# Ai00-X/ai00_server

Measured on NVIDIA H100. Metric: decode tokens/s RWKV-6-World-7B fp16 batch=16, higher is better.
Workload: dtype f16

## Files before the change

### ai00_server_b200/csrc/engine.cu

```cuda
#include "../../include/b200rwkv.h"

#include <unistd.h>

#include <algorithm>
#include <condition_variable>
#include <functional>
#include <thread>
#include <cmath>
#include <cstdio>
#include <cstdlib>
#include <cstring>
#include <map>
#include <memory>
#include <mutex>
#include <set>
#include <stdexcept>
#include <string>
#include <utility>
#include <vector>

#include "gemm.cuh"
#include "qgemm.cuh"
#include "pre6.cuh"
#include "sample.cuh"
// ... 572 lines not shown
    uint32_t ad_targets = 0;
    std::vector<AdLayer> ad_layers;
    GemmLaunch ad_head;
    AdapterParams s_head;
    int* d_slot_adapter = nullptr;
    std::vector<int> slot_adapter;
    struct AdMatrix {
        std::string name;
        int N, K;
        uint8_t* W;
        int tiles, KB, kbw;
        AdapterParams* sp;
        int proj;
        __half* A[AD_MAX];
    };
    std::vector<AdMatrix> ad_mats;
    std::vector<char> place_full;
    std::map<std::string, StTensor> model_shapes;
    uint8_t* ad_stage = nullptr;
    size_t ad_stage_cols = 0;
    void set_place_rank(const AdMatrix& m, int id, int r);
    void load_place(int id, const StFile& f, float alpha);
    void unload_place(int id);
    void drop_adapter_graphs();
    bool step_bound(const std::vector<int>& slots) const {
        for (int s : slots)
            if (n_adapters && s >= 0 && s < S && slot_adapter[s]) return true;
        return false;
    }
    GemmLaunch ad_launch(const GemmLaunch& base, AdapterParams& sp);
    void enqueue_shrink(const AdapterParams& p, const StepShape& sh, cudaStream_t s, Profiler* prof);
    void check_loras(const StFile& model) const;
    void blend_loras(const StTensor& t);

    Buf<__half> d_tmp;
    const StTensor* d_tmp_holds = nullptr;

    ~b200rwkv_engine();
    void* dalloc(size_t bytes, bool zero = true);
    void build(const StFile& st);
    const __half* upload_tmp(const StTensor& t);
    float* vec_f32(const StFile& st, const std::string& name, size_t off, size_t count, float scale = 1.f, float bias = 0.f);
    A16Buf a16_alloc(int K, int nmat = 1);
    GemmLaunch make_launch(std::vector<SegDesc>& segs, int force_grid = 0, int qtype = QT_NONE);
    int quant_layers = 0, quant_type = QT_NONE;
    int pick_split(int K, int tiles) const;
    void finalize_tp();
    template <typename P, typename... X>
    void launch_k(void (*kern)(P, X...), dim3 grid, dim3 block, size_t smem, const P& params, int cls, cudaStream_t s, Profiler* prof,
                  X... extra);
    bool split_on = false;
    bool split_act = false;
    bool ln_cluster_ok = false;
    unsigned* pre_gbar = nullptr;
    int launch_cluster = 0;
    unsigned long long* d_step_trace = nullptr;
    std::vector<int> step_trace_types;
    static constexpr int STEP_TRACE_MAX = 1024;
    static constexpr int STEP_TRACE_ROW = 512;
    bool trace_capture = false;
    std::vector<long long> step_trace_bytes;
    unsigned long long* tr_next(int label) {
        if (!d_step_trace || !trace_capture || launches_last_step >= STEP_TRACE_MAX) return nullptr;
        if ((int)step_trace_types.size() <= launches_last_step) step_trace_types.resize(launches_last_step + 1);
        step_trace_types[launches_last_step] = label;
        return d_step_trace + (size_t)STEP_TRACE_ROW * launches_last_step;
    }
    StepShape step_shape(int T, int R) const;
    void launch_gemm(const GemmLaunch& g, const StepShape& sh, cudaStream_t s, Profiler* prof, bool head = false);
    void launch_wkv(const WkvParams& p, const StepShape& sh, cudaStream_t s, Profiler* prof);
    LnPick launch_embed(const EmbedParams& p, const StepShape& sh, cudaStream_t s, Profiler* prof);
    LnPick launch_ln(const LnMixParams& p, const StepShape& sh, cudaStream_t s, Profiler* prof);
    LnPick launch_pre6(const Pre6Params& q, const StepShape& sh, cudaStream_t s, Profiler* prof);
    LnPick launch_ln_out(const LnOutParams& p, const StepShape& sh, cudaStream_t s, Profiler* prof);
    void enqueue_step(cudaStream_t s, const StepShape& sh, Profiler* prof);
    void run_step(const StepShape& sh);
    int fill_meta(int* m, const std::vector<int>& slots, const std::vector<int>& counts, const std::vector<const uint32_t*>& toks,
                  const std::vector<int>& outmode , int* R_out);
    struct ScoreOut { float* score; uint32_t* argmax; };
    void infer(int nslot, const int32_t* slot, const int32_t* ntok, const uint32_t* tokens, const int32_t* option,
               float* logits_out, size_t cap, int32_t* rows_out, const ScoreOut* score = nullptr, const SnapPlan* snap = nullptr);
    void state_xform(int slot, bool import, float* snap = nullptr);
};

b200rwkv_engine::~b200rwkv_engine() {
    cudaSetDevice(dev);
    cudaDeviceSynchronize();
    for (int q = 0; q < 8; ++q)
        if (peer_ipc[q] && peer_base[q]) cudaIpcCloseMemHandle(peer_base[q]);
}

void* b200rwkv_engine::dalloc(size_t bytes, bool zero) {
    bytes = std::max<size_t>(bytes, 16);
    allocs.emplace_back(bytes);
    if (zero) CK(cudaMemset(allocs.back(), 0, bytes));
    return allocs.back();
}

const __half* b200rwkv_engine::upload_tmp(const StTensor& t) {
    if (d_tmp_holds != &t) {
        REQUIRE(t.nbytes <= d_tmp.bytes, B200RWKV_ERR_INVALID, "internal: temp buffer too small");
        CK(cudaMemcpy(d_tmp, t.data, t.nbytes, cudaMemcpyHostToDevice));
        d_tmp_holds = &t;
        blend_loras(t);
    }
    return d_tmp;
}
// ... 401 lines not shown
    REQUIRE(H % world == 0 && F % (8 * world) == 0 && V % world == 0, B200RWKV_ERR_UNSUPPORTED,
            "heads / hidden / vocab do not shard evenly over the tensor-parallel world");
    Cl = C / world; Hl = H / world; Fl = F / world; Vl = V / world;
    const int ver = info.version;
    const int c0 = rank * Cl, f0 = rank * Fl, v0 = rank * Vl;

    stream = new_stream();
    sm_stream = new_stream();
    if (quant_layers > 0 && quant_type != QT_NONE) {
        REQUIRE(quant_type == QT_INT8 || quant_type == QT_NF4, B200RWKV_ERR_UNSUPPORTED, "quant_type must be Int8 or NF4 (SF4 is not implemented)");
        REQUIRE(world == 1, B200RWKV_ERR_UNSUPPORTED, "quantised layers are single-GPU in this version");
        REQUIRE(precision == 0, B200RWKV_ERR_UNSUPPORTED, "quantised layers run with precision 0 (f16 operands)");
    }
    gemm_smem_limits(quant_layers > 0 ? quant_type : (int)QT_NONE);
    wkv_smem_limits();
    if (precision == 1) split_act = true;

    meta_ints = MetaView::ints(maxT, S);
    d_meta = (int*)dalloc(meta_ints * 4);
    h_meta = HostBuf<int>(meta_ints * 4 * META_RING);
    memset(h_meta, 0, meta_ints * 4 * META_RING);
    for (auto& ev : meta_ev) ev = new_event(cudaEventDisableTiming);
    MetaView mv{d_meta, maxT, S};

    size_t tmp_bytes = 0;
    for (auto& kv : st.tensors) tmp_bytes = std::max(tmp_bytes, kv.second.nbytes);
    d_tmp = Buf<__half>(tmp_bytes);

    att_shift = (float*)dalloc((size_t)L * S * C * 4);
    ffn_shift = (float*)dalloc((size_t)L * S * C * 4);
    wkv_state = (float*)dalloc((size_t)L * S * Hl * N * N * 4);
    d_api = (float*)dalloc((size_t)L * (N + 2) * C * 4);
    state_from_st(st, L, H, N, C, init_state);

    const size_t TC = (size_t)maxT * C, TCl = (size_t)maxT * Cl;
    x_a = (float*)dalloc(TC * 4); x_b = (float*)dalloc(TC * 4);
    xx1 = (float*)dalloc(TC * 4); sx1 = (float*)dalloc(TC * 4); xx2 = (float*)dalloc(TC * 4);
    f_r = (float*)dalloc(TCl * 4); f_k = (float*)dalloc(TCl * 4); f_v = (float*)dalloc(TCl * 4); f_g = (float*)dalloc(TCl * 4);
    f_w = (float*)dalloc(TCl * 4); f_a = (float*)dalloc(TCl * 4); f_nu = (float*)dalloc(TCl * 4); f_vfirst = (float*)dalloc(TCl * 4);
    {
        auto al = [](size_t x) { return (x + 255) & ~(size_t)255; };
        off_part_att = 0;
        off_part_ffn = al(off_part_att + TC * 4 * 8);
        off_rr = al(off_part_ffn + TC * 4 * 8);
        off_logits = al(off_rr + TCl * 4);
        off_flags = al(off_logits + (size_t)maxT * Vl * 4);
        comm_bytes = al(off_flags + 256);
        comm_base = (uint8_t*)dalloc(comm_bytes, true);
        part_att = (float*)(comm_base + off_part_att);
        part_ffn = (float*)(comm_base + off_part_ffn);
        f_rr = (float*)(comm_base + off_rr);
        d_logits = (float*)(comm_base + off_logits);
        d_epoch = (unsigned*)dalloc(16, true);
        pre_gbar = (unsigned*)dalloc(256, true);
        ln_cluster_ok = ln_cluster_fits(C);
        split_on = split_act && ln_cluster_ok;
        REQUIRE(precision != 1 || split_on, B200RWKV_ERR_UNSUPPORTED, "precision 1 needs num_emb to be a multiple of 32 and <= 8192");
    }
    const int S_att = pick_split(Cl, cdiv(C, GEMM_BN)), S_ffn = pick_split(Fl, cdiv(C, GEMM_BN));
    split_att = S_att; split_ffn = S_ffn;
    d_hidden = (float*)dalloc(TC * 4);
    d_hid_tab = (float**)dalloc((size_t)L * sizeof(float*));
    step_done = new_event(cudaEventDisableTiming);
    keep_valid.assign(S, 0);
    if (rank == 0) {
        d_keep = (float*)dalloc((size_t)S * V * 4);
        const int nseg = cdiv(V, TOPK_SEG);
        if (nseg <= TOPK_MAX_SEGS) {
            tk_cand_x = (float*)dalloc((size_t)S * nseg * TOPK_MAX * 4);
            tk_cand_id = (unsigned*)dalloc((size_t)S * nseg * TOPK_MAX * 4);
            tk_stats = (float2*)dalloc((size_t)S * nseg * 8);
            tk_out_id = (unsigned*)dalloc((size_t)S * TOPK_MAX * 4);
            tk_out_p = (float*)dalloc((size_t)S * TOPK_MAX * 4);
        }
    }
    auto op_cols = [&](int K) { return n_adapters ? (cdiv(K, GEMM_BK) + n_adapters) * GEMM_BK : K; };
    for (int i = 0; i < 6; ++i) a_x[i] = a16_alloc(op_cols(C));
    a_out = a16_alloc(op_cols(Cl));
    a_kk = a16_alloc(op_cols(Fl));
    a_head = a16_alloc(op_cols(C));
    slot_adapter.assign(S, 0);
    if (n_adapters) d_slot_adapter = (int*)dalloc((size_t)S * 4, true);

    {
        const StTensor& e = st.get("emb.weight");
        emb = (__half*)dalloc(e.nbytes, false);
        CK(cudaMemcpy(emb, e.data, e.nbytes, cudaMemcpyHostToDevice));
        embed.emb = emb; embed.C = C; embed.V = V; embed.meta = mv;
        embed.ln_w = vec_f32(st, "blocks.0.ln0.weight", 0, C);
        embed.ln_b = vec_f32(st, "blocks.0.ln0.bias", 0, C);
        embed.x_out = x_a;
    }

    auto base_ln = [&](LnMixParams& p) {
        memset(&p, 0, sizeof(p));
        p.C = C; p.meta = mv;
    };
    auto f32_seg = [&](const StTensor& t, int n0, int Nn, int k0, int K, const A16Buf& ab, float* out, int ldo, int act,
                       const float* bias, int a_koff = 0, int a_mat = 0) {
        SegDesc d;
        d.t = &t; d.n0 = n0; d.N = Nn; d.k0 = k0; d.K = K;
        REQUIRE(a_koff % GEMM_BK == 0, B200RWKV_ERR_INVALID, "internal: split-K slices start on k-block boundaries");
        d.proto.A = ab.p + (size_t)a_mat * ab.halves_per_matrix + (size_t)(a_koff / GEMM_BK) * A16_KB_HALVES;
        d.proto.out_mode = OUT_F32; d.proto.act = act; d.proto.bias = bias; d.proto.out = out; d.proto.ldo = ldo;
        return d;
    };
    auto a16_seg = [&](const StTensor& t, int n0, int Nn, int k0, int K, const A16Buf& ab, const A16Buf& dst, int act,
// ... 47 lines not shown
            if (l == 0) {
                a_lora[0] = a16_alloc(Dm, 5);
                a_lora[1] = a16_alloc(Dd);
            }
            n1.n_mix = 1;
            n1.mu[0] = vec_f32(st, a + "time_mix_x", 0, C);
            n1.mix_out[0] = a_x[5].p;
            n1.sx_out = sx1;
            {
                std::vector<SegDesc> sv;
                SegDesc d = a16_seg(st.get(a + "time_mix_w1"), 0, 5 * Dm, 0, C, a_x[5], a_lora[0], ACT_TANH, nullptr);
                d.proto.grp = Dm;
                d.proto.grp_stride = (int)a_lora[0].halves_per_matrix;
                sv.push_back(d);
                ly.lora.push_back(make_launch(sv));
            }
            static const char* names[5] = {"time_mix_w", "time_mix_k", "time_mix_v", "time_mix_r", "time_mix_g"};
            const float* mu5[5];
            for (int i = 0; i < 5; ++i) mu5[i] = vec_f32(st, a + names[i], 0, C);
            {
                std::vector<SegDesc> sv;
                for (int i = 0; i < 5; ++i) {
                    SegDesc d;
                    d.t = &st.get(a + "time_mix_w2"); d.slice = i; d.n0 = 0; d.N = C; d.k0 = 0; d.K = Dm;
                    d.proto.A = a_lora[0].p + (size_t)i * a_lora[0].halves_per_matrix;
                    d.proto.out_mode = OUT_LERP_A16; d.proto.act = ACT_NONE;
                    d.proto.out = a_x[i].p;
                    d.proto.aux0 = xx1; d.proto.aux1 = sx1; d.proto.aux2 = mu5[i]; d.proto.ld_aux = C;
                    sv.push_back(d);
                }
                ly.lora.push_back(make_launch(sv));
            }
            {
                const StTensor& w1 = st.get(a + "time_mix_w1");
                const StTensor& w2 = st.get(a + "time_mix_w2");
                const StTensor& d2 = st.get(a + "time_decay_w2");
                REQUIRE(w1.shape.size() == 2 && w1.shape[0] == 5 * Dm && w1.shape[1] == C, B200RWKV_ERR_INVALID, "time_mix_w1 must be [5*Dm, C]");
                REQUIRE(w2.shape.size() == 3 && w2.shape[0] == 5 && w2.shape[1] == C && w2.shape[2] == Dm, B200RWKV_ERR_INVALID,
                        "time_mix_w2 must be [5, C, Dm]");
                REQUIRE(d2.shape.size() == 2 && d2.shape[0] == C && d2.shape[1] == Dd, B200RWKV_ERR_INVALID, "time_decay_w2 must be [C, Dd]");
            }
            if (pre6_fits(Dm, C)) {
                auto upload_raw = [&](const StTensor& t) {
                    __half* d = (__half*)dalloc(t.nbytes, false);
                    CK(cudaMemcpy(d, t.data, t.nbytes, cudaMemcpyHostToDevice));
                    return d;
                };
                Pre6Params& q = ly.pre6;
                q.W1 = upload_raw(st.get(a + "time_mix_w1"));
                q.W2 = upload_raw(st.get(a + "time_mix_w2"));
                for (int i = 0; i < 5; ++i) { q.mu[i] = mu5[i]; q.out[i] = a_x[i].p; }
                q.lora = a_lora[0].p; q.lora_stride = (int)a_lora[0].halves_per_matrix;
                q.Dm = Dm;
                q.gbar = pre_gbar;
                ly.has_pre6 = true;
            }
            {
                std::vector<SegDesc> sv;
                sv.push_back(f32_seg(Wr, c0, Cl, 0, C, a_x[3], f_r, Cl, ACT_NONE, nullptr));
                sv.push_back(f32_seg(Wk, c0, Cl, 0, C, a_x[1], f_k, Cl, ACT_NONE, nullptr));
                sv.push_back(f32_seg(Wv, c0, Cl, 0, C, a_x[2], f_v, Cl, ACT_NONE, nullptr));
                sv.push_back(f32_seg(st.get(a + "gate.weight"), c0, Cl, 0, C, a_x[4], f_g, Cl, ACT_SILU, nullptr));
                if (lq != QT_NONE) {
                    std::vector<SegDesc> sd;
                    sd.push_back(a16_seg(st.get(a + "time_decay_w1"), 0, Dd, 0, C, a_x[0], a_lora[1], ACT_TANH, nullptr));
                    ly.pre.push_back(make_launch(sd));
                    ly.pre.push_back(make_launch(sv, 0, lq));
                } else {
                    sv.push_back(a16_seg(st.get(a + "time_decay_w1"), 0, Dd, 0, C, a_x[0], a_lora[1], ACT_TANH, nullptr));
                    ly.pre.push_back(make_launch(sv));
                }
            }
            const float* time_decay = vec_f32(st, a + "time_decay", c0, Cl);
            if (Dd <= 128 && Dd % 8 == 0) {
                const StTensor& t = st.get(a + "time_decay_w2");
                const std::vector<__half> tmp = wd2_k_major(reinterpret_cast<const __half*>(t.data), c0, Hl, Dd);
                __half* dw = (__half*)dalloc(tmp.size() * 2, false);
                CK(cudaMemcpy(dw, tmp.data(), tmp.size() * 2, cudaMemcpyHostToDevice));
                wk.wd2t = dw;
                wk.decay_bias = time_decay;
                wk.d1 = a_lora[1].p;
                wk.Dd = Dd;
            } else {
                std::vector<SegDesc> sv;
                sv.push_back(f32_seg(st.get(a + "time_decay_w2"), c0, Cl, 0, Dd, a_lora[1], f_w, Cl, ACT_EXPNEGEXP, time_decay));
                ly.pre.push_back(make_launch(sv));
            }
            wk.w = f_w;
            wk.u = vec_f32(st, a + "time_first", c0, Cl);
        } else if (ver == 5) {
            static const char* names[4] = {"time_mix_k", "time_mix_v", "time_mix_r", "time_mix_g"};
            n1.n_mix = 4;
            for (int i = 0; i < 4; ++i) {
                n1.mu[i] = vec_f32(st, a + names[i], 0, C, -1.f, 1.f);
                n1.mix_out[i] = a_x[1 + i].p;
            }
            std::vector<SegDesc> sv;
            sv.push_back(f32_seg(Wr, c0, Cl, 0, C, a_x[3], f_r, Cl, ACT_NONE, nullptr));
            sv.push_back(f32_seg(Wk, c0, Cl, 0, C, a_x[1], f_k, Cl, ACT_NONE, nullptr));
            sv.push_back(f32_seg(Wv, c0, Cl, 0, C, a_x[2], f_v, Cl, ACT_NONE, nullptr));
            sv.push_back(f32_seg(st.get(a + "gate.weight"), c0, Cl, 0, C, a_x[4], f_g, Cl, ACT_SILU, nullptr));
            ly.pre.push_back(make_launch(sv, 0, lq));
            {
                const StTensor& td = st.get(a + "time_decay");
                REQUIRE(td.numel() == C, B200RWKV_ERR_UNSUPPORTED, "v5 time_decay must be [H, N]");
                float* d = (float*)dalloc((size_t)Cl * 4, false);
                Buf<__half> tmp((size_t)Cl * 2);
// ... 1917 lines not shown
                "gate blocks (C / n_gate columns) must be whole multiples of 4 columns");
        REQUIRE(!x.commit_src == !x.commit_dst, B200RWKV_ERR_INVALID, "the commit needs both commit_src and commit_dst");
    }
    if (stage == 1 || stage == 2) {
        REQUIRE(x.n_mix >= 1 && x.n_mix <= 6, B200RWKV_ERR_INVALID, "n_mix must be 1..6");
        REQUIRE(x.shift_state && x.mu && x.mix_out && x.xx_out, B200RWKV_ERR_INVALID, "null shift_state, mu, mix_out or xx_out");
        REQUIRE(x.x_out || x.n_parts == 0, B200RWKV_ERR_INVALID, "in place (x_out NULL) takes no parts");
    }
    if (stage == 2) {
        REQUIRE(T <= 16 && pre6_fits(x.Dm, C), B200RWKV_ERR_UNSUPPORTED,
                "the front half runs decode-shaped steps (T <= 16) with Dm 32 or 64, C % 128 == 0 and C <= 4096");
        REQUIRE(x.n_mix == 1 && x.sx_out && x.W1 && x.W2 && x.mu5 && x.lora_out && x.out5, B200RWKV_ERR_INVALID,
                "the front half needs n_mix 1, sx_out, W1, W2, mu5, lora_out and out5");
    }
    std::vector<int> outmode(x.nslot, 0);
    if (stage == 3) {
        REQUIRE(x.option && x.head_out, B200RWKV_ERR_INVALID, "ln_out needs option and head_out");
        for (int i = 0; i < x.nslot; ++i) {
            REQUIRE(x.option[i] >= B200RWKV_OPTION_LAST && x.option[i] <= B200RWKV_OPTION_NONE, B200RWKV_ERR_INVALID, "bad option");
            outmode[i] = x.option[i] == B200RWKV_OPTION_FULL ? 2 : (x.option[i] == B200RWKV_OPTION_LAST ? 1 : 0);
        }
    }
    snap_args_ok(x.nsnap, x.snap_tok, x.snap_rec, x.snap_ld, x.snap_off, C, T);
    if (x.nsnap > 0) {
        REQUIRE(stage != 0, B200RWKV_ERR_INVALID, "the embed stage takes no snapshots");
        REQUIRE(NL == 1, B200RWKV_ERR_INVALID, "snapshots take one launch");
        REQUIRE(stage != 3 || (x.commit_src && x.snap_head_out), B200RWKV_ERR_INVALID, "ln_out snapshots need the commit and snap_head_out");
    }

    st.start(device, NL, x.tokens, outmode);
    float* d_rec = x.nsnap > 0 ? st.snap_start(x.nsnap, x.snap_tok, x.snap_rec, x.snap_ld) : nullptr;
    b200rwkv_engine* e = st.e.get();
    e->ln_cluster_ok = ln_cluster_fits(C);
    const StepShape& sh = st.sh;
    const int th = sh.th;
    const int hrows = std::max(sh.th_rows, 16);
    const int xrows = sh.split ? 32 : 16 * sh.MTX;

    auto rows_down = [&](float* h, const float* d) { CK(cudaMemcpy(h, d, (size_t)T * C * 4, cudaMemcpyDeviceToHost)); };
    auto a16_up = [&](const uint16_t* h, int nmat, int K, int tr) {
        const std::vector<uint16_t> b = a16_pack(h, nmat * K, K, tr, (size_t)tr * K, K);
        return (__half*)st.up(b.data(), b.size() * 2);
    };
    auto a16_down = [&](uint16_t* h, const __half* d, int nmat, int K, int tr) {
        std::vector<uint16_t> b(a16_halves(K) * nmat);
        CK(cudaMemcpy(b.data(), d, b.size() * 2, cudaMemcpyDeviceToHost));
        a16_unpack(b, nmat * K, K, tr, tr, (size_t)tr * K, K, h);
    };

    const size_t TC = (size_t)T * C;
    const float* ln_w = (const float*)st.up(x.ln_w, (size_t)C * 4);
    const float* ln_b = (const float*)st.up(x.ln_b, (size_t)C * 4);
    float* cdst = x.commit_dst ? (float*)st.up(x.commit_dst, (size_t)S * C * 4) : nullptr;
    unsigned* gbar = (unsigned*)e->dalloc(256, true);
    float** hid_tab = nullptr;
    std::vector<float*> hid_rows(NL, nullptr);
    const int gcl = x.n_gate > 0 ? C / x.n_gate : 0;
    auto residual = [&](auto& p, int l) {
        p.x_in = st.rows_up(x.x_in + l * TC, C);
        p.C = C;
        p.meta = st.meta(l);
        p.n_parts = x.n_parts;
        for (int q = 0; q < x.n_parts; ++q) p.parts[q] = st.rows_up(x.parts + ((size_t)l * x.n_parts + q) * TC, C);
        p.n_gate = x.n_gate;
        p.gate_cl = gcl;
        for (int q = 0; q < x.n_gate; ++q) p.gates[q] = st.rows_up(x.gates + ((size_t)l * x.n_gate + q) * T * gcl, gcl);
        p.ln_w = ln_w; p.ln_b = ln_b;
        p.commit_dst = cdst;
        p.commit_src = x.commit_src ? st.rows_up(x.commit_src + l * TC, C) : nullptr;
        if (x.hidden) hid_rows[l] = st.rows_up(x.hidden + l * TC, C);
    };

    std::vector<EmbedParams> em(NL);
    std::vector<LnMixParams> lm(NL);
    std::vector<Pre6Params> pq(NL);
    std::vector<LnOutParams> lo(NL);
    if (stage == 0) {
        const __half* emb = (const __half*)st.up(x.emb, (size_t)x.V * C * 2);
        for (int l = 0; l < NL; ++l) {
            EmbedParams& p = em[l];
            memset(&p, 0, sizeof(p));
            p.emb = emb; p.C = C; p.V = x.V; p.meta = st.meta(l);
            p.ln_w = ln_w; p.ln_b = ln_b;
            p.x_out = st.rows_up(x.x_out + l * TC, C);
        }
    } else if (stage == 1 || stage == 2) {
        const float* shift = (const float*)st.up(x.shift_state, (size_t)S * C * 4);
        const float* mu = (const float*)st.up(x.mu, (size_t)x.n_mix * C * 4);
        if (x.hidden) hid_tab = (float**)e->dalloc((size_t)NL * sizeof(float*), true);
        for (int l = 0; l < NL; ++l) {
            LnMixParams& p = lm[l];
            memset(&p, 0, sizeof(p));
            residual(p, l);
            p.x_out = x.x_out ? st.rows_up(x.x_out + l * TC, C) : const_cast<float*>(p.x_in);
            p.shift_state = shift;
            p.n_mix = x.n_mix;
            const __half* mix = a16_up(x.mix_out + (size_t)l * x.n_mix * th * C, x.n_mix, C, th);
            for (int j = 0; j < x.n_mix; ++j) { p.mu[j] = mu + (size_t)j * C; p.mix_out[j] = const_cast<__half*>(mix) + j * a16_halves(C); }
            p.xx_out = st.rows_up(x.xx_out + l * TC, C);
            p.sx_out = x.sx_out ? st.rows_up(x.sx_out + l * TC, C) : nullptr;
            p.hid_slot = hid_tab ? hid_tab + l : nullptr;
            p.snap_rec = st.snap_table; p.snap_off = (size_t)x.snap_off;
        }
        if (hid_tab) CK(cudaMemcpy(hid_tab, hid_rows.data(), (size_t)NL * sizeof(float*), cudaMemcpyHostToDevice));
        if (stage == 2) {
            const int Dm = x.Dm;
            const __half* W1 = (const __half*)st.up(x.W1, (size_t)5 * Dm * C * 2);
            const __half* W2 = (const __half*)st.up(x.W2, (size_t)5 * C * Dm * 2);
            const float* mu5 = (const float*)st.up(x.mu5, (size_t)5 * C * 4);
            for (int l = 0; l < NL; ++l) {
                Pre6Params& q = pq[l];
                memset(&q, 0, sizeof(q));
                q.ln = lm[l];
                q.W1 = W1; q.W2 = W2;
                const __half* o5 = a16_up(x.out5 + (size_t)l * 5 * th * C, 5, C, th);
                for (int j = 0; j < 5; ++j) { q.mu[j] = mu5 + (size_t)j * C; q.out[j] = const_cast<__half*>(o5) + j * a16_halves(C); }
                q.lora = const_cast<__half*>(a16_up(x.lora_out + (size_t)l * 5 * th * Dm, 5, Dm, th));
                q.lora_stride = (int)a16_halves(Dm);
                q.Dm = Dm;
                q.gbar = gbar;
            }
        }
    } else {
        for (int l = 0; l < NL; ++l) {
            LnOutParams& p = lo[l];
            memset(&p, 0, sizeof(p));
            residual(p, l);
            p.head_in = const_cast<__half*>(a16_up(x.head_out + (size_t)l * hrows * C, 1, C, hrows));
            p.hidden_out = hid_rows[l];
            p.snap_rec = st.snap_table; p.snap_off = (size_t)x.snap_off;
            if (sh.MTX > 0) {
                p.snap_meta = st.snap_meta;
                p.snap_head_in = const_cast<__half*>(a16_up(x.snap_head_out, 1, C, xrows));
            }
        }
    }
    CK(cudaDeviceSynchronize());
    LnPick pick{};
    for (int l = 0; l < NL; ++l) {
        if (stage == 0) pick = e->launch_embed(em[l], sh, e->stream, nullptr);
        else if (stage == 1) pick = e->launch_ln(lm[l], sh, e->stream, nullptr);
        else if (stage == 2) pick = e->launch_pre6(pq[l], sh, e->stream, nullptr);
        else pick = e->launch_ln_out(lo[l], sh, e->stream, nullptr);
    }
    CK(cudaGetLastError());
    CK(cudaStreamSynchronize(e->stream));
    for (int l = 0; l < NL; ++l) {
        if (stage == 0) { rows_down(x.x_out + l * TC, em[l].x_out); continue; }
        if (x.hidden) rows_down(x.hidden + l * TC, hid_rows[l]);
        if (stage == 3) {
            a16_down(x.head_out + (size_t)l * hrows * C, lo[l].head_in, 1, C, hrows);
            if (lo[l].snap_head_in) a16_down(x.snap_head_out, lo[l].snap_head_in, 1, C, xrows);
            continue;
        }
        const LnMixParams& p = lm[l];
        if (x.x_out) rows_down(x.x_out + l * TC, p.x_out);
        else rows_down(x.x_in + l * TC, p.x_in);
        rows_down(x.xx_out + l * TC, p.xx_out);
        if (x.sx_out) rows_down(x.sx_out + l * TC, p.sx_out);
        a16_down(x.mix_out + (size_t)l * x.n_mix * th * C, p.mix_out[0], x.n_mix, C, th);
        if (stage == 2) {
            a16_down(x.out5 + (size_t)l * 5 * th * C, pq[l].out[0], 5, C, th);
            a16_down(x.lora_out + (size_t)l * 5 * th * x.Dm, pq[l].lora, 5, x.Dm, th);
        }
    }
    if (cdst) CK(cudaMemcpy(x.commit_dst, cdst, (size_t)S * C * 4, cudaMemcpyDeviceToHost));
    if (d_rec) CK(cudaMemcpy(x.snap_rec, d_rec, (size_t)x.nsnap * x.snap_ld * 4, cudaMemcpyDeviceToHost));
    if (x.kernel_out) { x.kernel_out[0] = pick.kernel; x.kernel_out[1] = pick.variant; x.kernel_out[2] = pick.split; }
    API_END
}

int32_t b200rwkv_op_gemm(int32_t device, int32_t T, int32_t precision, int32_t quant_type, int32_t grid, int32_t launches,
                         int32_t nseg, const b200rwkv_gemm_seg* seg, int32_t* plan_out) {
// ... 787 lines not shown
```

### ai00_server_b200/csrc/pre6.cuh

```cuda
#pragma once
#include <cooperative_groups.h>

#include "mix.cuh"

namespace b200 {
namespace cg = cooperative_groups;

constexpr int PRE_CLUSTER = 8;
constexpr int PRE_NCLUSTER = 16;
constexpr int PRE_GRID = PRE_CLUSTER * PRE_NCLUSTER;
constexpr int PRE_THREADS = 256;
constexpr int PRE_MAX_C = 4096;
constexpr int PRE_NT2 = 3;
constexpr int PRE_KSW = 4;
constexpr int PRE_TILES3 = 3;

struct Pre6Params {
    LnMixParams ln;
    const __half* W1;
    const __half* W2;
    const float* mu[5];
    __half* lora;
    int lora_stride;
    int lora_kq;
    __half* out[5];
    int Dm;
    unsigned* gbar;
};

__device__ __forceinline__ void mma_16816(float (&d)[4], const uint32_t (&a)[4], const uint32_t b0, const uint32_t b1) {
    asm volatile(
        "mma.sync.aligned.m16n8k16.row.col.f32.f16.f16.f32 {%0,%1,%2,%3}, {%4,%5,%6,%7}, {%8,%9}, {%0,%1,%2,%3};"
        : "+f"(d[0]), "+f"(d[1]), "+f"(d[2]), "+f"(d[3])
        : "r"(a[0]), "r"(a[1]), "r"(a[2]), "r"(a[3]), "r"(b0), "r"(b1));
}

__device__ __forceinline__ void pre_grid_barrier(cg::cluster_group& cl, const unsigned rank, unsigned* mine, unsigned* reset_before,
                                                 unsigned* reset_after, const unsigned tag) {
    cl.sync();
    if (rank == 0 && threadIdx.x == 0) {
        if (blockIdx.x == 0 && reset_before) st_relaxed_gpu(reset_before, 0u);
        red_add_release_gpu(mine, 1u);
        SpinGuard sg_;
        unsigned seen;
        while ((seen = ld_acquire_gpu(mine)) < (unsigned)PRE_NCLUSTER) sg_.poll(WD_GRIDBAR, 0x600u + tag, seen, blockIdx.x);
        if (blockIdx.x == 0 && reset_after) st_relaxed_gpu(reset_after, 0u);
        __threadfence();
    }
    cl.sync();
}

__device__ __forceinline__ float cluster_sum(cg::cluster_group& cl, const unsigned rank, float* xch, const float v) {
    if (threadIdx.x < PRE_CLUSTER) cl.map_shared_rank(xch, threadIdx.x)[rank] = v;
    cl.sync();
    float s = 0.f;
#pragma unroll
    for (int i = 0; i < PRE_CLUSTER; ++i) s += xch[i];
    return s;
}

__device__ __forceinline__ float4 residual_vec(const ResidualSrc& r, const int t, const int c) {
    const size_t base = (size_t)t * r.C + c;
    float4 a = ld4(r.x_in + base);
    if (r.n_parts == 0) return a;
    float4 v[8];
#pragma unroll
    for (int q = 0; q < 8; ++q) v[q] = (q < r.n_parts) ? ld4(r.parts[q] + base) : make_float4(0.f, 0.f, 0.f, 0.f);
    float4 gt = make_float4(1.f, 1.f, 1.f, 1.f);
    if (r.n_gate > 0) {
        const int gb = c / r.gate_cl;
        const float* gp = r.gates[0];
#pragma unroll
        for (int i = 1; i < 8; ++i) gp = (gb == i) ? r.gates[i] : gp;
        gt = ld4(gp + (size_t)t * r.gate_cl + (c - gb * r.gate_cl));
    }
    float4 s = make_float4(0.f, 0.f, 0.f, 0.f);
#pragma unroll
    for (int q = 0; q < 8; ++q) add4(s, v[q]);
    if (r.n_gate > 0) { s.x *= gt.x; s.y *= gt.y; s.z *= gt.z; s.w *= gt.w; }
    add4(a, s);
    return a;
}

__device__ __forceinline__ void slice_stats(cg::cluster_group& cl, const unsigned rank, const int C, const bool act, const float4 a,
                                            float* red, float* xch, float& mean, float& rstd) {
    const int Cs = C / PRE_CLUSTER;
    const float s = act ? (a.x + a.y) + (a.z + a.w) : 0.f;
    const float mi = block_sum(s, red) / (float)Cs;
    float s2 = 0.f;
    if (act) {
        const float dx = a.x - mi, dy = a.y - mi, dz = a.z - mi, dw = a.w - mi;
        s2 = (dx * dx + dy * dy) + (dz * dz + dw * dw);
    }
    const float m2i = block_sum(s2, red);
    if (threadIdx.x < PRE_CLUSTER) {
        float* dst = cl.map_shared_rank(xch, threadIdx.x);
        dst[rank] = mi;
        dst[PRE_CLUSTER + rank] = m2i;
    }
    cl.sync();
    float ms = 0.f;
#pragma unroll
// ... 3 lines not shown
#pragma unroll
    for (int i = 0; i < PRE_CLUSTER; ++i) {
        const float d = xch[i] - mean;
        m2 += xch[PRE_CLUSTER + i] + (float)Cs * d * d;
    }
    rstd = 1.0f / sqrtf(m2 / (float)C + LN_EPS);
}

template <int NMIX>
struct PreLnStatic {
    float4 w, b;
    float4 mu[NMIX];
    int T, slot, prev_t, last;
    float* hid;
    float* snap;
};

template <int NMIX>
__device__ __forceinline__ PreLnStatic<NMIX> pre_ln_static(const LnMixParams& p, const int t, const unsigned rank) {
    const int Cs = p.C / PRE_CLUSTER;
    PreLnStatic<NMIX> st;
    st.T = p.meta.T();
    st.slot = p.meta.tok_slot()[t];
    st.prev_t = p.meta.tok_prev()[t];
    st.last = p.meta.tok_last()[t];
    st.hid = p.hid_slot ? *p.hid_slot : nullptr;
    st.snap = (p.snap_rec && p.commit_dst && t < st.T) ? p.snap_rec[t] : nullptr;
    const bool act = 4 * (int)threadIdx.x < Cs;
    const int c = act ? (int)rank * Cs + 4 * (int)threadIdx.x : 0;
    const float4 z4 = make_float4(0.f, 0.f, 0.f, 0.f);
    st.w = act ? ld4(p.ln_w + c) : z4;
    st.b = act ? ld4(p.ln_b + c) : z4;
#pragma unroll
    for (int m = 0; m < NMIX; ++m) st.mu[m] = (act && m < p.n_mix) ? ld4(p.mu[m] + c) : z4;
    return st;
}

template <int NMIX, bool SPLIT = false>
__device__ __forceinline__ void pre_ln_slice(const LnMixParams& p, const int t, cg::cluster_group& cl, const unsigned rank,
                                             const PreLnStatic<NMIX>& st, float* red, float (*xch)[2 * PRE_CLUSTER]) {
    const int C = p.C, Cs = C / PRE_CLUSTER;
    const bool act = 4 * (int)threadIdx.x < Cs;
    const int c = act ? (int)rank * Cs + 4 * (int)threadIdx.x : 0;
    const int slot = st.slot, prev_t = st.prev_t;
    const bool last = st.last != 0;
    const ResidualSrc r = make_residual_src(p);
    const float4 z4 = make_float4(0.f, 0.f, 0.f, 0.f);
    float4 pv = z4, cm = z4;
    if (act && prev_t < 0) pv = ld4(p.shift_state + (size_t)slot * C + c);
    const bool commit = act && last && p.commit_dst;
    const bool snap = act && st.snap;
    if (commit || snap) cm = ld4(p.commit_src + (size_t)t * C + c);
    float4 a = act ? residual_vec(r, t, c) : z4;
    if (act && (p.x_out != p.x_in || p.n_parts > 0)) *reinterpret_cast<float4*>(p.x_out + (size_t)t * C + c) = a;
    if (act && st.hid) *reinterpret_cast<float4*>(st.hid + (size_t)t * C + c) = a;
    float mean, rstd;
    slice_stats(cl, rank, C, act, a, red, xch[0], mean, rstd);
    if (prev_t >= 0) {
        float pmean, prstd;
        pv = act ? residual_vec(r, prev_t, c) : z4;
        slice_stats(cl, rank, C, act, pv, red, xch[1], pmean, prstd);
        pv = ln_apply(pv, pmean, prstd, st.w, st.b);
    }
    if (!act) return;
    a = ln_apply(a, mean, rstd, st.w, st.b);
    float4 sx;
    sx.x = pv.x - a.x; sx.y = pv.y - a.y; sx.z = pv.z - a.z; sx.w = pv.w - a.w;
    *reinterpret_cast<float4*>(p.xx_out + (size_t)t * C + c) = a;
    if (p.sx_out) *reinterpret_cast<float4*>(p.sx_out + (size_t)t * C + c) = sx;
    if (commit) *reinterpret_cast<float4*>(p.commit_dst + (size_t)slot * C + c) = cm;
    if (snap) *reinterpret_cast<float4*>(st.snap + p.snap_off + c) = cm;
#pragma unroll
    for (int m = 0; m < NMIX; ++m) {
        if (m < p.n_mix) {
            const float4 mu = st.mu[m];
            if (SPLIT) {
                uint2 hi, lo;
                split_pack_h2(a.x + sx.x * mu.x, a.y + sx.y * mu.y, hi.x, lo.x);
                split_pack_h2(a.z + sx.z * mu.z, a.w + sx.w * mu.w, hi.y, lo.y);
                *reinterpret_cast<uint2*>(p.mix_out[m] + a16_index(t, c, 32)) = hi;
                *reinterpret_cast<uint2*>(p.mix_out[m] + a16_index(t + 16, c, 32)) = lo;
            } else {
                uint2 o;
                o.x = pack_h2(a.x + sx.x * mu.x, a.y + sx.y * mu.y);
                o.y = pack_h2(a.z + sx.z * mu.z, a.w + sx.w * mu.w);
                *reinterpret_cast<uint2*>(p.mix_out[m] + a16_index(t, c, 16)) = o;
            }
        }
    }
}

template <bool SPLIT = false>
__global__ void __launch_bounds__(PRE_THREADS) ln_mix_cluster_kernel(const __grid_constant__ LnMixParams p) {
    __shared__ float red[32];
    __shared__ float xch[2][2 * PRE_CLUSTER];
    cg::cluster_group cl = cg::this_cluster();
    const unsigned rank = cl.block_rank();
    const int t = blockIdx.x / PRE_CLUSTER;
    trace_stamp(p.trace, 0);
    pdl_launch_dependents();
    const PreLnStatic<6> st = pre_ln_static<6>(p, t, rank);
    cl.sync();
    pdl_wait();
    trace_stamp(p.trace, 1);
    if (t >= st.T) return;
    pre_ln_slice<6, SPLIT>(p, t, cl, rank, st, red, xch);
    cl.sync();
    trace_stamp(p.trace, 7);
}

template <int KD, bool SPLIT = false>
__global__ void __launch_bounds__(PRE_THREADS, 2) pre6_kernel(const __grid_constant__ Pre6Params p) {
    __shared__ float red[32];
    __shared__ float xch[2][2 * PRE_CLUSTER];
    __shared__ __align__(16) float red2[8][PRE_NT2 * 4 * 32];
    __shared__ float part[PRE_NT2 * 4 * 32];
    cg::cluster_group cl = cg::this_cluster();
    const unsigned rank = cl.block_rank();
    const int g = blockIdx.x / PRE_CLUSTER;
    const int tid = threadIdx.x, warp = tid >> 5, lane = tid & 31, grp = lane >> 2, tig = lane & 3;
    constexpr int Dm = KD * 16;
    constexpr int TH = SPLIT ? 32 : 16;
    constexpr int NR = 5 * Dm;
    constexpr int RG = (NR + PRE_NCLUSTER - 1) / PRE_NCLUSTER;
    static_assert(RG <= PRE_NT2 * 8, "row group does not fit the n-tiles");
    const int C = p.ln.C, Cs = C / PRE_CLUSTER;
    unsigned long long* const tr = p.ln.trace;
    trace_stamp(tr, 0);
    auto cta_stamp = [&](int i) {
        if (tr && threadIdx.x == 0) tr[8 + 3 * blockIdx.x + i] = globaltimer_ns();
    };
    cta_stamp(0);
    pdl_launch_dependents();

    const PreLnStatic<1> st = pre_ln_static<1>(p.ln, g, rank);
    uint32_t w1f[PRE_KSW][PRE_NT2][2];
    const int ksteps = Cs / 16;
#pragma unroll
    for (int i = 0; i < PRE_KSW; ++i) {
        const int kstep = warp + 8 * i;
        const int kb = (int)rank * Cs + kstep * 16 + tig * 2;
#pragma unroll
        for (int nt = 0; nt < PRE_NT2; ++nt) {
            const int nrow = nt * 8 + grp, n = g * RG + nrow;
            const bool ok = kstep < ksteps && nrow < RG && n < NR;
            const __half* src = p.W1 + (size_t)n * C + kb;
            w1f[i][nt][0] = ok ? *reinterpret_cast<const uint32_t*>(src) : 0u;
            w1f[i][nt][1] = ok ? *reinterpret_cast<const uint32_t*>(src + 8) : 0u;
        }
    }
    const int nchunks = C / 8;
    const int cpc = (nchunks + PRE_GRID - 1) / PRE_GRID;
    const int ch_lo = min((int)blockIdx.x * cpc, nchunks), ch_hi = min(ch_lo + cpc, nchunks);
    const int nch = ch_hi - ch_lo, ntiles = nch * 5;
    uint32_t w2f[PRE_TILES3][KD][2];
    float2 mu3[PRE_TILES3];
    int tj[PRE_TILES3], tc0[PRE_TILES3];
#pragma unroll
    for (int i = 0; i < PRE_TILES3; ++i) {
        const int q = warp + 8 * i;
        const bool ok = q < ntiles;
        const int j = ok ? q / nch : 0, ci = ok ? q - j * nch : 0;
        tj[i] = ok ? j : -1;
        tc0[i] = (ch_lo + ci) * 8;
        const __half* src = p.W2 + ((size_t)j * C + tc0[i] + grp) * Dm + tig * 2;
#pragma unroll
        for (int ks = 0; ks < KD; ++ks) {
            w2f[i][ks][0] = ok ? *reinterpret_cast<const uint32_t*>(src + ks * 16) : 0u;
            w2f[i][ks][1] = ok ? *reinterpret_cast<const uint32_t*>(src + ks * 16 + 8) : 0u;
        }
        mu3[i] = ok ? *reinterpret_cast<const float2*>(p.mu[j] + tc0[i] + tig * 2) : make_float2(0.f, 0.f);
    }
    cl.sync();
    pdl_wait();
    trace_stamp(tr, 1);
    cta_stamp(1);
    const int T = min(st.T, 16);

    if (g < T) pre_ln_slice<1, SPLIT>(p.ln, g, cl, rank, st, red, xch);
    trace_stamp(tr, 2);
    cta_stamp(2);
    pre_grid_barrier(cl, rank, p.gbar, p.gbar + 32, nullptr, 1);
    trace_stamp(tr, 3);

    {
        float acc[PRE_NT2][4];
#pragma unroll
        for (int nt = 0; nt < PRE_NT2; ++nt)
#pragma unroll
            for (int e = 0; e < 4; ++e) acc[nt][e] = 0.f;
#pragma unroll
        for (int sp = 0; sp < (SPLIT ? 2 : 1); ++sp) {
            const __half* xa = p.ln.mix_out[0];
            uint32_t af[PRE_KSW][4];
#pragma unroll
            for (int i = 0; i < PRE_KSW; ++i) {
                const int kstep = warp + 8 * i;
                const int k = (int)rank * Cs + kstep * 16;
                const uint32_t* src = reinterpret_cast<const uint32_t*>(xa + a16_index(16 * sp + grp, k + tig * 2, TH));
                const bool ok = kstep < ksteps;
                af[i][0] = ok ? __ldcg(src) : 0u;
                af[i][1] = ok ? __ldcg(src + 32) : 0u;
                af[i][2] = ok ? __ldcg(src + TH * 4) : 0u;
                af[i][3] = ok ? __ldcg(src + TH * 4 + 32) : 0u;
            }
#pragma unroll
            for (int i = 0; i < PRE_KSW; ++i)
#pragma unroll
                for (int nt = 0; nt < PRE_NT2; ++nt) mma_16816(acc[nt], af[i], w1f[i][nt][0], w1f[i][nt][1]);
        }
#pragma unroll
        for (int nt = 0; nt < PRE_NT2; ++nt)
#pragma unroll
            for (int e = 0; e < 4; ++e) red2[warp][(nt * 4 + e) * 32 + lane] = acc[nt][e];
        __syncthreads();
        for (int o = tid; o < PRE_NT2 * 4 * 32; o += PRE_THREADS) {
            float s = 0.f;
#pragma unroll
            for (int w = 0; w < 8; ++w) s += red2[w][o];
            part[o] = s;
        }
        cl.sync();
        constexpr int PER = PRE_NT2 * 4 * 32 / PRE_CLUSTER;
        if (tid < PER) {
            const int o = (int)rank * PER + tid;
            float v[PRE_CLUSTER];
#pragma unroll
            for (int r = 0; r < PRE_CLUSTER; ++r) v[r] = cl.map_shared_rank(part, r)[o];
            float s = 0.f;
#pragma unroll
            for (int r = 0; r < PRE_CLUSTER; ++r) s += v[r];
            const int nt = o / 128, e = (o >> 5) & 3, ln = o & 31;
            const int t = (ln >> 2) + ((e & 2) ? 8 : 0);
            const int nrow = nt * 8 + (ln & 3) * 2 + (e & 1);
            const int n = g * RG + nrow;
            if (t < T && nrow < RG && n < NR) {
                const int j = n / Dm, nn = n - j * Dm;
                __half* dst = p.lora + (size_t)j * p.lora_stride;
                if (SPLIT) {
                    __half hi, lo;
                    split_h(apply_act(s, ACT_TANH), hi, lo);
                    dst[a16_index(t, nn, TH)] = hi;
                    dst[a16_index(t + 16, nn, TH)] = lo;
                } else {
                    dst[a16_index(t, nn, TH)] = f2h_sat(apply_act(s, ACT_TANH));
                }
            }
        }
    }
    trace_stamp(tr, 4);
    pre_grid_barrier(cl, rank, p.gbar + 32, nullptr, p.gbar, 2);

    trace_stamp(tr, 5);
    {
        uint32_t af[PRE_TILES3][KD][4];
        float2 xx[PRE_TILES3][2], sx[PRE_TILES3][2];
        float acc3[SPLIT ? PRE_TILES3 : 1][4];
        if (SPLIT) {
#pragma unroll
            for (int i = 0; i < PRE_TILES3; ++i)
#pragma unroll
                for (int e = 0; e < 4; ++e) acc3[SPLIT ? i : 0][e] = 0.f;
#pragma unroll
            for (int i = 0; i < PRE_TILES3; ++i) {
                const bool ok = tj[i] >= 0;
                const uint32_t* src = reinterpret_cast<const uint32_t*>(p.lora + (size_t)(ok ? tj[i] : 0) * p.lora_stride +
                                                                        a16_index(16 + grp, tig * 2, TH));
#pragma unroll
                for (int ks = 0; ks < KD; ++ks) {
                    af[i][ks][0] = ok ? __ldcg(src + ks * TH * 8) : 0u;
                    af[i][ks][1] = ok ? __ldcg(src + ks * TH * 8 + 32) : 0u;
                    af[i][ks][2] = ok ? __ldcg(src + ks * TH * 8 + TH * 4) : 0u;
                    af[i][ks][3] = ok ? __ldcg(src + ks * TH * 8 + TH * 4 + 32) : 0u;
                }
            }
#pragma unroll
            for (int i = 0; i < PRE_TILES3; ++i)
#pragma unroll
                for (int ks = 0; ks < KD; ++ks) mma_16816(acc3[SPLIT ? i : 0], af[i][ks], w2f[i][ks][0], w2f[i][ks][1]);
        }
#pragma unroll
        for (int i = 0; i < PRE_TILES3; ++i) {
            const bool ok = tj[i] >= 0;
            const uint32_t* src = reinterpret_cast<const uint32_t*>(p.lora + (size_t)(ok ? tj[i] : 0) * p.lora_stride + a16_index(grp, tig * 2, TH));
#pragma unroll
            for (int ks = 0; ks < KD; ++ks) {
                af[i][ks][0] = ok ? __ldcg(src + ks * TH * 8) : 0u;
                af[i][ks][1] = ok ? __ldcg(src + ks * TH * 8 + 32) : 0u;
                af[i][ks][2] = ok ? __ldcg(src + ks * TH * 8 + TH * 4) : 0u;
                af[i][ks][3] = ok ? __ldcg(src + ks * TH * 8 + TH * 4 + 32) : 0u;
            }
#pragma unroll
            for (int h = 0; h < 2; ++h) {
                const int t = grp + 8 * h;
                const size_t at = (size_t)t * C + tc0[i] + tig * 2;
                const bool okt = ok && t < T;
                xx[i][h] = okt ? __ldcg(reinterpret_cast<const float2*>(p.ln.xx_out + at)) : make_float2(0.f, 0.f);
                sx[i][h] = okt ? __ldcg(reinterpret_cast<const float2*>(p.ln.sx_out + at)) : make_float2(0.f, 0.f);
            }
        }
#pragma unroll
        for (int i = 0; i < PRE_TILES3; ++i) {
            if (tj[i] < 0) continue;
            float acc[4] = {0.f, 0.f, 0.f, 0.f};
            if (SPLIT) {
#pragma unroll
                for (int e = 0; e < 4; ++e) acc[e] = acc3[SPLIT ? i : 0][e];
            }
#pragma unroll
            for (int ks = 0; ks < KD; ++ks) mma_16816(acc, af[i][ks], w2f[i][ks][0], w2f[i][ks][1]);
            __half* outp = p.out[tj[i]];
#pragma unroll
            for (int h = 0; h < 2; ++h) {
                const int t = grp + 8 * h;
                if (t >= T) continue;
                const float y0 = xx[i][h].x + sx[i][h].x * (mu3[i].x + acc[2 * h]);
                const float y1 = xx[i][h].y + sx[i][h].y * (mu3[i].y + acc[2 * h + 1]);
                if (SPLIT) {
                    uint32_t hi, lo;
                    split_pack_h2(y0, y1, hi, lo);
                    *reinterpret_cast<uint32_t*>(outp + a16_index(t, tc0[i] + tig * 2, TH)) = hi;
                    *reinterpret_cast<uint32_t*>(outp + a16_index(t + 16, tc0[i] + tig * 2, TH)) = lo;
                } else {
                    *reinterpret_cast<uint32_t*>(outp + a16_index(t, tc0[i] + tig * 2, TH)) = pack_h2(y0, y1);
                }
            }
        }
    }    trace_stamp(tr, 7);
}

}
```

Before: 2285.

## Replace pre6 grid barriers with per-cluster and per-mix dependency flags

Replaces the two full grid barriers in the fused pre6 kernel. The first becomes a per-slice counter shared by clusters of the same rank. The second becomes per-LoRA-matrix counters, so each tile waits only for the groups that produce its mix, and the final cluster sync is split into an arrive/wait pair. It also hoists the xx/sx loads ahead of the wait and defers the residual stores until after the stats reduction. This is meant to cut barrier stall time in each layer's prologue, at the cost of more complex flag epoch logic with subtle ordering and reset risks.

```diff
diff --git a/ai00_server_b200/csrc/engine.cu b/ai00_server_b200/csrc/engine.cu
--- a/ai00_server_b200/csrc/engine.cu
+++ b/ai00_server_b200/csrc/engine.cu
@@ -648,7 +648,7 @@
     bool split_on = false;
     bool split_act = false;
     bool ln_cluster_ok = false;
-    unsigned* pre_gbar = nullptr;
+    unsigned* pre_flags = nullptr;
     int launch_cluster = 0;
     unsigned long long* d_step_trace = nullptr;
     std::vector<int> step_trace_types;
@@ -1156,7 +1156,7 @@
         f_rr = (float*)(comm_base + off_rr);
         d_logits = (float*)(comm_base + off_logits);
         d_epoch = (unsigned*)dalloc(16, true);
-        pre_gbar = (unsigned*)dalloc(256, true);
+        pre_flags = (unsigned*)dalloc(PRE_FLAG_BYTES, true);
         ln_cluster_ok = ln_cluster_fits(C);
         split_on = split_act && ln_cluster_ok;
         REQUIRE(precision != 1 || split_on, B200RWKV_ERR_UNSUPPORTED, "precision 1 needs num_emb to be a multiple of 32 and <= 8192");
@@ -1310,7 +1310,7 @@
                 for (int i = 0; i < 5; ++i) { q.mu[i] = mu5[i]; q.out[i] = a_x[i].p; }
                 q.lora = a_lora[0].p; q.lora_stride = (int)a_lora[0].halves_per_matrix;
                 q.Dm = Dm;
-                q.gbar = pre_gbar;
+                q.flags = pre_flags;
                 ly.has_pre6 = true;
             }
             {
@@ -3334,7 +3334,7 @@
     const float* ln_w = (const float*)st.up(x.ln_w, (size_t)C * 4);
     const float* ln_b = (const float*)st.up(x.ln_b, (size_t)C * 4);
     float* cdst = x.commit_dst ? (float*)st.up(x.commit_dst, (size_t)S * C * 4) : nullptr;
-    unsigned* gbar = (unsigned*)e->dalloc(256, true);
+    unsigned* flags = (unsigned*)e->dalloc(PRE_FLAG_BYTES, true);
     float** hid_tab = nullptr;
     std::vector<float*> hid_rows(NL, nullptr);
     const int gcl = x.n_gate > 0 ? C / x.n_gate : 0;
@@ -3400,7 +3400,7 @@
                 q.lora = const_cast<__half*>(a16_up(x.lora_out + (size_t)l * 5 * th * Dm, 5, Dm, th));
                 q.lora_stride = (int)a16_halves(Dm);
                 q.Dm = Dm;
-                q.gbar = gbar;
+                q.flags = flags;
             }
         }
     } else {
diff --git a/ai00_server_b200/csrc/pre6.cuh b/ai00_server_b200/csrc/pre6.cuh
--- a/ai00_server_b200/csrc/pre6.cuh
+++ b/ai00_server_b200/csrc/pre6.cuh
@@ -25,8 +25,19 @@
     int lora_kq;
     __half* out[5];
     int Dm;
-    unsigned* gbar;
+    unsigned* flags;
 };
+
+struct PreFlags {
+    static constexpr int LINE = 32;
+    unsigned* f;
+    __device__ __forceinline__ unsigned* xhat(int s) const { return f + LINE * s; }
+    __device__ __forceinline__ unsigned* lora(int j) const { return f + LINE * (PRE_CLUSTER + j); }
+};
+constexpr size_t PRE_FLAG_BYTES = (size_t)(PRE_CLUSTER + 5) * PreFlags::LINE * 4;
+
+__device__ __forceinline__ void cluster_arrive_relaxed() { asm volatile("barrier.cluster.arrive.relaxed.aligned;" ::: "memory"); }
+__device__ __forceinline__ void cluster_wait() { asm volatile("barrier.cluster.wait.acquire.aligned;" ::: "memory"); }
 
 __device__ __forceinline__ void mma_16816(float (&d)[4], const uint32_t (&a)[4], const uint32_t b0, const uint32_t b1) {
     asm volatile(
@@ -35,19 +46,9 @@
         : "r"(a[0]), "r"(a[1]), "r"(a[2]), "r"(a[3]), "r"(b0), "r"(b1));
 }
 
-__device__ __forceinline__ void pre_grid_barrier(cg::cluster_group& cl, const unsigned rank, unsigned* mine, unsigned* reset_before,
-                                                 unsigned* reset_after, const unsigned tag) {
-    cl.sync();
-    if (rank == 0 && threadIdx.x == 0) {
-        if (blockIdx.x == 0 && reset_before) st_relaxed_gpu(reset_before, 0u);
-        red_add_release_gpu(mine, 1u);
-        SpinGuard sg_;
-        unsigned seen;
-        while ((seen = ld_acquire_gpu(mine)) < (unsigned)PRE_NCLUSTER) sg_.poll(WD_GRIDBAR, 0x600u + tag, seen, blockIdx.x);
-        if (blockIdx.x == 0 && reset_after) st_relaxed_gpu(reset_after, 0u);
-        __threadfence();
-    }
-    cl.sync();
+__host__ __device__ constexpr int pre_mix_g_lo(int j, int Dm, int RG) { return j * Dm / RG; }
+__host__ __device__ constexpr int pre_mix_g_hi(int j, int Dm, int RG) {
+    return ((j + 1) * Dm - 1) / RG < PRE_NCLUSTER - 1 ? ((j + 1) * Dm - 1) / RG : PRE_NCLUSTER - 1;
 }
 
 __device__ __forceinline__ float cluster_sum(cg::cluster_group& cl, const unsigned rank, float* xch, const float v) {
@@ -157,8 +158,6 @@
     const bool snap = act && st.snap;
     if (commit || snap) cm = ld4(p.commit_src + (size_t)t * C + c);
     float4 a = act ? residual_vec(r, t, c) : z4;
-    if (act && (p.x_out != p.x_in || p.n_parts > 0)) *reinterpret_cast<float4*>(p.x_out + (size_t)t * C + c) = a;
-    if (act && st.hid) *reinterpret_cast<float4*>(st.hid + (size_t)t * C + c) = a;
     float mean, rstd;
     slice_stats(cl, rank, C, act, a, red, xch[0], mean, rstd);
     if (prev_t >= 0) {
@@ -168,6 +167,8 @@
         pv = ln_apply(pv, pmean, prstd, st.w, st.b);
     }
     if (!act) return;
+    if (p.x_out != p.x_in || p.n_parts > 0) *reinterpret_cast<float4*>(p.x_out + (size_t)t * C + c) = a;
+    if (st.hid) *reinterpret_cast<float4*>(st.hid + (size_t)t * C + c) = a;
     a = ln_apply(a, mean, rstd, st.w, st.b);
     float4 sx;
     sx.x = pv.x - a.x; sx.y = pv.y - a.y; sx.z = pv.z - a.z; sx.w = pv.w - a.w;
@@ -260,21 +261,22 @@
     const int nch = ch_hi - ch_lo, ntiles = nch * 5;
     uint32_t w2f[PRE_TILES3][KD][2];
     float2 mu3[PRE_TILES3];
-    int tj[PRE_TILES3], tc0[PRE_TILES3];
+    int tj[PRE_TILES3];
+    auto tile_c0 = [&](int i) { const int q = warp + 8 * i; return (ch_lo + q - (q / nch) * nch) * 8; };
 #pragma unroll
     for (int i = 0; i < PRE_TILES3; ++i) {
         const int q = warp + 8 * i;
         const bool ok = q < ntiles;
         const int j = ok ? q / nch : 0, ci = ok ? q - j * nch : 0;
         tj[i] = ok ? j : -1;
-        tc0[i] = (ch_lo + ci) * 8;
-        const __half* src = p.W2 + ((size_t)j * C + tc0[i] + grp) * Dm + tig * 2;
+        const int c0 = (ch_lo + ci) * 8;
+        const __half* src = p.W2 + ((size_t)j * C + c0 + grp) * Dm + tig * 2;
 #pragma unroll
         for (int ks = 0; ks < KD; ++ks) {
             w2f[i][ks][0] = ok ? *reinterpret_cast<const uint32_t*>(src + ks * 16) : 0u;
             w2f[i][ks][1] = ok ? *reinterpret_cast<const uint32_t*>(src + ks * 16 + 8) : 0u;
         }
-        mu3[i] = ok ? *reinterpret_cast<const float2*>(p.mu[j] + tc0[i] + tig * 2) : make_float2(0.f, 0.f);
+        mu3[i] = ok ? *reinterpret_cast<const float2*>(p.mu[j] + c0 + tig * 2) : make_float2(0.f, 0.f);
     }
     cl.sync();
     pdl_wait();
@@ -285,7 +287,17 @@
     if (g < T) pre_ln_slice<1, SPLIT>(p.ln, g, cl, rank, st, red, xch);
     trace_stamp(tr, 2);
     cta_stamp(2);
-    pre_grid_barrier(cl, rank, p.gbar, p.gbar + 32, nullptr, 1);
+    __syncthreads();
+    if (tid == 0) {
+        if (blockIdx.x == 0)
+            for (int j = 0; j < 5; ++j) st_relaxed_gpu(PreFlags{p.flags}.lora(j), 0u);
+        unsigned* const xc = PreFlags{p.flags}.xhat((int)rank);
+        const unsigned target = (atom_add_acq_rel_gpu(xc, 1u) & ~(unsigned)(PRE_NCLUSTER - 1)) + PRE_NCLUSTER;
+        SpinGuard sg_;
+        unsigned seen;
+        while ((int)((seen = ld_acquire_gpu(xc)) - target) < 0) sg_.poll(WD_GRIDBAR, 0x610u + rank, seen, blockIdx.x);
+    }
+    __syncthreads();
     trace_stamp(tr, 3);
 
     {
@@ -353,13 +365,39 @@
             }
         }
     }
+    __syncthreads();
+    if (tid == 0) {
+        const int j_lo = g * RG / Dm, j_hi = min(((g + 1) * RG - 1) / Dm, 4);
+        for (int j = j_lo; j <= j_hi; ++j) red_add_release_gpu(PreFlags{p.flags}.lora(j), 1u);
+    }
+    cluster_arrive_relaxed();
     trace_stamp(tr, 4);
-    pre_grid_barrier(cl, rank, p.gbar + 32, nullptr, p.gbar, 2);
-
+
+    float2 xx[PRE_TILES3][2], sx[PRE_TILES3][2];
+#pragma unroll
+    for (int i = 0; i < PRE_TILES3; ++i) {
+#pragma unroll
+        for (int h = 0; h < 2; ++h) {
+            const int t = grp + 8 * h;
+            const bool okt = tj[i] >= 0 && t < T;
+            const size_t at = okt ? (size_t)t * C + tile_c0(i) + tig * 2 : 0;
+            xx[i][h] = okt ? __ldcg(reinterpret_cast<const float2*>(p.ln.xx_out + at)) : make_float2(0.f, 0.f);
+            sx[i][h] = okt ? __ldcg(reinterpret_cast<const float2*>(p.ln.sx_out + at)) : make_float2(0.f, 0.f);
+        }
+    }
+
+#pragma unroll
+    for (int i = 0; i < PRE_TILES3; ++i) {
+        const int j = tj[i];
+        if (j < 0) continue;
+        const unsigned want = (unsigned)(PRE_CLUSTER * (pre_mix_g_hi(j, Dm, RG) - pre_mix_g_lo(j, Dm, RG) + 1));
+        SpinGuard sg_;
+        unsigned seen;
+        while ((seen = ld_acquire_gpu(PreFlags{p.flags}.lora(j))) < want) sg_.poll(WD_GRIDBAR, 0x620u + j, seen, blockIdx.x);
+    }
     trace_stamp(tr, 5);
     {
         uint32_t af[PRE_TILES3][KD][4];
-        float2 xx[PRE_TILES3][2], sx[PRE_TILES3][2];
         float acc3[SPLIT ? PRE_TILES3 : 1][4];
         if (SPLIT) {
 #pragma unroll
@@ -394,14 +432,6 @@
                 af[i][ks][1] = ok ? __ldcg(src + ks * TH * 8 + 32) : 0u;
                 af[i][ks][2] = ok ? __ldcg(src + ks * TH * 8 + TH * 4) : 0u;
                 af[i][ks][3] = ok ? __ldcg(src + ks * TH * 8 + TH * 4 + 32) : 0u;
-            }
-#pragma unroll
-            for (int h = 0; h < 2; ++h) {
-                const int t = grp + 8 * h;
-                const size_t at = (size_t)t * C + tc0[i] + tig * 2;
-                const bool okt = ok && t < T;
-                xx[i][h] = okt ? __ldcg(reinterpret_cast<const float2*>(p.ln.xx_out + at)) : make_float2(0.f, 0.f);
-                sx[i][h] = okt ? __ldcg(reinterpret_cast<const float2*>(p.ln.sx_out + at)) : make_float2(0.f, 0.f);
             }
         }
 #pragma unroll
@@ -424,14 +454,16 @@
                 if (SPLIT) {
                     uint32_t hi, lo;
                     split_pack_h2(y0, y1, hi, lo);
-                    *reinterpret_cast<uint32_t*>(outp + a16_index(t, tc0[i] + tig * 2, TH)) = hi;
-                    *reinterpret_cast<uint32_t*>(outp + a16_index(t + 16, tc0[i] + tig * 2, TH)) = lo;
+                    *reinterpret_cast<uint32_t*>(outp + a16_index(t, tile_c0(i) + tig * 2, TH)) = hi;
+                    *reinterpret_cast<uint32_t*>(outp + a16_index(t + 16, tile_c0(i) + tig * 2, TH)) = lo;
                 } else {
-                    *reinterpret_cast<uint32_t*>(outp + a16_index(t, tc0[i] + tig * 2, TH)) = pack_h2(y0, y1);
+                    *reinterpret_cast<uint32_t*>(outp + a16_index(t, tile_c0(i) + tig * 2, TH)) = pack_h2(y0, y1);
                 }
             }
         }
-    }    trace_stamp(tr, 7);
-}
-
-}
+    }
+    cluster_wait();
+    trace_stamp(p.ln.trace, 7);
+}
+
+}
```

New measurement: 2301, median of 6. Within noise of the previous version (+0.7%).
